# omroot/DeepLearningInAssetPricing_PaperReplication

Measured on AMD Instinct MI355X. Metric: epochs/sec (3-phase GAN), higher is better.
Workload: dtype bf16; 1 GPU; model=Chen-Pelger-Zhu GAN: LSTM[4] + SDF FFN[64,64] + 8 tanh moments, global_batch=1, seq_len=240, panel=T=240/60/300 N=3000 F=46 M=178, bench_config=real, wide_layer0=False, models_per_gpu=1, parallelism=ensemble-dp1, backend=none

## Files before the change

csrc/engine.cpp:

```cpp
#include <cstdint>
#include <cstdlib>
#include <hip/hip_runtime.h>
#include <pybind11/numpy.h>
#include <pybind11/pybind11.h>
#include <pybind11/stl.h>

#include <execinfo.h>
#include <signal.h>
#include <sys/syscall.h>
#include <unistd.h>

#include <atomic>
#include <cmath>
#include <cstring>
#include <map>
#include <memory>
#include <mutex>
#include <stdexcept>
#include <string>
#include <vector>

#include <chrono>

#include "engine_plan.h"
// ... 137 lines not shown
    {
      hipDeviceProp_t prop;
      int dev = 0;
      HIP_OK(hipGetDevice(&dev));
      HIP_OK(hipGetDeviceProperties(&prop, dev));
      std::vector<uint32_t> mask((prop.multiProcessorCount + 31) / 32, 0u);
      for (int cu = 0; cu < prop.multiProcessorCount; ++cu) mask[cu / 32] |= 1u << (cu % 32);
      HIP_OK(hipExtStreamCreateWithCUMask(&st2_, (uint32_t)mask.size(), mask.data()));
    }
    own_st_ = st_;
    for (hipEvent_t& e : ev_) HIP_OK(hipEventCreateWithFlags(&e, hipEventDisableTiming));
    build_desc(F, M, nrnn, H, raw_macro_sdf, hidden, mom_hidden, K, dropout, normalize_w, weighted,
               residual, fp32);
    prog_.alloc((size_t)G * 3 * 16);
    esync_.alloc(64);
    d_desc_.alloc(sizeof(ModelDesc));
    HIP_LEGACY(hipMemcpy(d_desc_.p, &md_, sizeof(ModelDesc), hipMemcpyHostToDevice));
    models_.resize(G);
    for (int g = 0; g < G; ++g) {
      ModelState& S = models_[g];
      S.dropout = dropout;
      S.params.alloc(md_.P); S.grads.alloc(md_.P); S.m.alloc(md_.P); S.v.alloc(md_.P);
      S.snap_loss.alloc(md_.P); S.snap_sharpe.alloc(md_.P);
      S.gnorm.alloc(1); S.best.alloc(3); S.aux.alloc((size_t)2 * md_.md.aux_floats);
      S.hist.alloc((size_t)max_epochs_ * HIST_W);
      S.adam_step.alloc(2); S.drop_step.alloc(1); S.snap_flags.alloc(2); S.ep.alloc(2); S.upd_ctr.alloc(1);
      S.tail_ctr.alloc(lstm_tail_words());
      S.blob.alloc((size_t)2 * md_.md.blob_frags * 512 * xw());
      S.blob0.alloc((size_t)std::max(1, md_.md.b0_frags) * 512 * xw());
      S.wproj.alloc((size_t)(md_.proj_mp + 2) * md_.proj_np);
// ... 846 lines not shown
  }
  EvalPass eval_pass(int phase) const {
    EvalPass ep;
    ep.gram = gram_eval() && plan_ev_[phase];
    return ep;
  }
  const LossJob* loss_tab(int phase, bool gram) const {
    return gram ? as<LossJob>(j_loss_gram_[phase]) : as<LossJob>(j_loss_train_[phase]);
  }
  double capture_s_ = 0.0;
  double host_launch_s_ = 0.0;
  long host_launch_n_ = 0;
  DevBuf<char> j_rnn_all_;
  DevBuf<int> prog_;
  DevBuf<int> esync_;
  int cap_train_ = 0, cap_eval_ = 0, cap_all_ = 0;
  int tail_cap_ = 0;
  PhasePlan plan_[4];
  static int fused_grid(int want, int njobs, int cap) {
    if (cap <= 0 || njobs <= 0) return 0;
    const int gx = std::min(want, cap / njobs - 1);
    return gx >= 16 ? gx : 0;
  }
  int eval_grid() const {
    int gx = std::max(gx_fwd_[1], gx_fwd_[2]);
    if (k_.eval_gx > 0) gx = std::min(gx, k_.eval_gx);
    return gx;
  }
  int train_fwd_grid(int phase) const { return phase == 2 ? gx_fwd_[0] : gx_fwd13_; }
  int ne_per_model() const { return G_ > 0 && n_eval_jobs_ % G_ == 0 ? n_eval_jobs_ / G_ : 0; }
// ... 12 lines not shown
      p.eval_gx_solo = eval_gx;
      p.eval_fusable = eval_fusable;
      const int gx = fused_grid(train_fwd_grid(phase), G_, cap_train_);
      p.fused_fwd = (phase != 2 || k_.fused_p2) && overlap && fits(splits_[0].T) && gx > 0;
      p.train_gx = p.fused_fwd ? gx : 0;
      p.selfproj = p.fused_fwd && k_.self_proj && !train_mom(phase);
      const int gxa = cap_all_ > 0 && ne > 0 ? std::min(train_fwd_grid(phase), cap_all_ / G_ - 1 - ne) : 0;
      p.eval_in_fwd = k_.eval_in_fwd && phase != 2 && ne > 0 && p.fused_fwd && fits(tmax_fwd_all()) && gxa >= 16;
      p.all_gx = p.eval_in_fwd ? gxa : 0;
      p.sep_eval = k_.eval_sep && phase != 2 && p.fused_fwd && eval_fusable;
      p.tail_fused = k_.fused_tail && !xs_on_ && phase != 2 && have0 && lstm_tail_supported(md_, splits_[0].T);
      const int nadam = (md_.P_sdf + ADAM_PB - 1) / ADAM_PB;
      p.adam_in_tail = k_.tail_adam != 0 && !safe_mode_ && p.tail_fused && packs && tail_cap_ > 0 &&
                       2 * G_ * nadam <= tail_cap_;
      p.split_graphs = k_.split_graphs && !safe_mode_ && p.adam_in_tail && (p.sep_eval || p.eval_in_fwd);
      p.mom_tail = phase == 2 && k_.mom_tail && !xs_on_ && packs && have0 && mom_tail_supported(md_, splits_[0].T);
      p.p2_lstm_cached = phase == 2 && k_.p2_lstm_cache && md_.nrnn > 0 && (md_.nrnn == 1 || md_.dropout == 0.f) &&
                         !xs_on_;
      plan_[phase] = p;
    }
  }
  RunMode run_mode(int phase) const {
    const PhasePlan& p = plan_[phase];
    RunMode m;
    m.pipe = phase != 2 && n_eval_jobs_ > 0 && pipeline_;
    m.split = m.pipe && p.split_graphs;
    m.sep = m.split && p.sep_eval;
    m.tail_adam = m.split || (m.pipe && p.eval_in_fwd && k_.tail_adam == 2 && p.adam_in_tail);
    return m;
  }
 public:
  double capture_seconds() const { return capture_s_; }
  bool fused_fwd(int phase) const { return phase >= 1 && phase <= 3 && plan_[phase].fused_fwd; }
  void reset_prog_errors() {
    sync();
    std::vector<int> h((size_t)G_ * 3 * 16);
    HIP_LEGACY(hipMemcpy(h.data(), prog_.p, h.size() * sizeof(int), hipMemcpyDeviceToHost));
    for (int k = 0; k < 3 * G_; ++k) h[16 * k + 1] = 0;
    HIP_LEGACY(hipMemcpy(prog_.p, h.data(), h.size() * sizeof(int), hipMemcpyHostToDevice));
    for (ModelState& S : models_) {
      HIP_LEGACY(hipMemset(S.tail_ctr.p, 0, S.tail_ctr.n * sizeof(int)));
      HIP_LEGACY(hipMemset(S.upd_ctr.p, 0, S.upd_ctr.n * sizeof(int)));
    }
    HIP_LEGACY(hipMemset(esync_.p, 0, esync_.n * sizeof(int)));
  }
  py::dict fused_info() const {
    py::dict d;
    const RunMode m = run_mode(1);
    d["cap_train"] = cap_train_; d["cap_eval"] = cap_eval_;
    for (int ph = 1; ph <= 3; ++ph) d[("train_gx_p" + std::to_string(ph)).c_str()] = plan_[ph].train_gx;
    d["eval_gx_solo"] = plan_[1].eval_gx_solo;
    d["cap_all"] = cap_all_;
    d["tail_cap"] = tail_cap_;
    for (int ph = 1; ph <= 3; ph += 2) {
      d[("eval_in_fwd_p" + std::to_string(ph)).c_str()] = plan_[ph].eval_in_fwd;
      d[("all_gx_p" + std::to_string(ph)).c_str()] = plan_[ph].all_gx;
    }
    d["eval_per_model"] = ne_per_model();
    d["fused_tail"] = plan_[1].tail_fused;
    d["mom_tail"] = plan_[2].mom_tail;
    d["p2_lstm_cached"] = plan_[2].p2_lstm_cached;
    d["adam_in_tail"] = m.tail_adam && plan_[1].eval_in_fwd;
    d["split_graphs"] = m.split;
    d["eval_sep"] = m.sep;
    d["host_launch_us_per_epoch"] = host_launch_n_ ? 1e6 * host_launch_s_ / host_launch_n_ : 0.0;
    d["bwd_nfine"] = nfine_; d["bwd_fpw"] = fpw_;
    d["fused_pack"] = inv_code_.p != nullptr;
    d["bwd_lds_fpw1"] = (long)mlp_bwd_lds_bytes(md_.md, slab_stride(), 1);
    d["bwd_lds_fpw4"] = (long)mlp_bwd_lds_bytes(md_.md, slab_stride(), 4);
    return d;
  }
  int prog_timeouts() {
    sync();
    std::vector<int> h((size_t)G_ * 3 * 16);
    HIP_LEGACY(hipMemcpy(h.data(), prog_.p, h.size() * sizeof(int), hipMemcpyDeviceToHost));
    int n = 0;
    for (int k = 0; k < 3 * G_; ++k) n += h[16 * k + 1];
    return n;
  }
// ... 450 lines not shown
  }
  void join_eval_gram() {
    if (!eval_gram_pending_) return;
    HIP_OK(hipStreamWaitEvent(st_, ev_[EV_GRAM], 0));
    eval_gram_pending_ = false;
  }

  void rebuild_jobs() {
    HTRACE("rebuild_jobs");
    sync();
    if (st2_) HIP_OK(hipStreamSynchronize(st2_));
    for (ModelState& S : models_) {
      HIP_LEGACY(hipMemset(S.tail_ctr.p, 0, S.tail_ctr.n * sizeof(int)));
      HIP_LEGACY(hipMemset(S.upd_ctr.p, 0, S.upd_ctr.n * sizeof(int)));
    }
    tail_cap_ = splits_[0].set && lstm_tail_supported(md_, splits_[0].T) ? lstm_tail_capacity(md_, splits_[0].T) : 0;
    for (auto& kv : graphs_) retire_graph_exec(kv.second, st_);
    graphs_.clear();
    fwd_tables_.clear();
    j_mlp_bwd_dh_.free();
    {
      const int want = k_.bwd_fpw;
      const int tps = std::max(md_.tps_s, md_.tps_m);
      fpw_ = (want == 4 && !md_.tbwd && mlp_bwd_fpw_fits(md_.md, md_.KS1, slab_stride(), tps, 4)) ? 4 : 1;
      gx_bwd_ = nfine_ / fpw_;
    }
    std::vector<RnnJob> rt, re;
    std::vector<LossJob> le, led;
    std::vector<MlpJob> me;
    std::vector<FinJob> fj;
// ... 298 lines not shown
      HTRACE("launch_mlp_fwd_zx");
      launch_mlp_fwd_zx(as<MlpJob>(j_mlp_eval_), n_eval_jobs_, std::max(1, k_.zx_gx / n_eval_jobs_), md_.md, md_.WMB, st);
    } else {
      if (md_.md.wide)
        launch_proj0(as<WideJob>(j_wide_eval_), n_eval_jobs_, std::max(gx_proj_[1], gx_proj_[2]), md_.md, md_.WMB, st);
      HTRACE("launch_mlp_fwd");
      if (fused_eval(ep))
        launch_mlp_fwd_rnn(as<MlpJob>(j_mlp_eval_), as<RnnJob>(j_rnn_eval_), dd(), n_eval_jobs_, plan_[1].eval_gx_solo,
                           md_.md, md_.KS1, md_.WMB, md_.H, md_.nrnn, tmax_eval_, st, k_.h_cache, 0, ep.selfproj);
      else
        launch_mlp_fwd(as<MlpJob>(j_mlp_eval_), n_eval_jobs_, eval_grid(), md_.md, md_.KS1, md_.WMB, st, k_.h_cache);
    }
    const LossJob* le = as<LossJob>(ep.gram ? j_loss_eval_ : j_loss_eval_dense_);
    HTRACE("launch_period_fwd");
    period_fwd(le, n_eval_jobs_, tmax_eval_, st, false, 6);
    if (ep.gram) {
      HTRACE("launch_period_bwd(eval)");
      launch_period_bwd(le, n_eval_jobs_, tmax_eval_, st);
    } else {
      HTRACE("launch_asset");
      launch_asset(le, n_eval_jobs_, nmax_eval_, md_.K, st);
      if (xs_on_) { launch_xs_loss_sums(le, n_eval_jobs_, st); xs_call("loss", 6, st); }
    }
    HTRACE("launch_job_metrics");
    launch_job_metrics(le, n_eval_jobs_, st);
  }
  void enqueue_eval_solo(int phase) {
    EvalPass ep = eval_pass(phase);
    ep.solo = true;
    enqueue_eval(st_, ep);
  }
  void enqueue_epoch_end(int phase, int ignore_epoch, float sel, hipStream_t st, int signal = 0) {
    HTRACE("launch_epoch_end");
    launch_epoch_end(as<EpochJob>(j_epoch_[phase]), G_, phase, ignore_epoch, sel, md_.residual_factor,
                     md_.P, st, signal);
  }
  void enqueue_epoch(int phase, float lr, int ignore_epoch, float sel, bool lstm_once) {
    TrainPass tp = epoch_pass(phase, lr);
    tp.mom_adam = plan_[phase].mom_tail;
    tp.lstm_once = lstm_once;
    enqueue_train_grads(tp);
    if (!tp.mom_adam) enqueue_update(phase, lr);
    if (phase != 2) enqueue_eval_solo(phase);
    enqueue_epoch_end(phase, ignore_epoch, sel, st_);
  }
  void enqueue_head(int phase, float lr, int part) {
    TrainPass tp = epoch_pass(phase, lr);
    tp.part = part;
    enqueue_train_grads(tp);
    enqueue_dropmask(phase, 1, st_);
// ... 10 lines not shown
    tp.esig = sep ? nullptr : esync_.p;
    enqueue_train_grads(tp);
  }
  void enqueue_eval_split(int phase, int ignore_epoch, float sel) {
    EvalPass ep = eval_pass(phase);
    if (plan_[phase].sep_eval) {
      HTRACE("launch_wait_gen");
      launch_wait_gen(as<UpdJob>(j_upd_), G_, k_.spin_limit, st2_);
      ep.sep = true;
      ep.selfproj = k_.self_proj && k_.h_cache;
      if (!ep.selfproj) launch_proj(as<RnnJob>(j_rnn_eval_), n_eval_jobs_, tmax_eval_, dd(), md_, st2_, !k_.h_cache);
    } else {
      HTRACE("launch_wait_count");
      launch_wait_count(esync_.p, ne_per_model() * G_, k_.spin_limit, prog_.p, G_, st2_);
    }
    enqueue_eval_towers(st2_, ep);
    enqueue_dropmask(phase, 1, st2_);
    enqueue_epoch_end(phase, ignore_epoch, sel, st2_, 1);
  }
  void enqueue_pipe(int phase, float lr, int ignore_epoch, float sel) {
    HIP_OK(hipEventRecord(ev_[EV_FORK], st_));
    HIP_OK(hipStreamWaitEvent(st2_, ev_[EV_FORK], 0));
    TrainPass tp = epoch_pass(phase, lr);
    tp.premasked = true;
    const EvalPass ep = eval_pass(phase);
    if (plan_[phase].eval_in_fwd) {
      const bool ta = run_mode(phase).tail_adam;
      tp.eval_rnn = tp.mark_fwd = tp.tail_metrics = true;
      tp.tail_adam = ta ? 2 : 0;
      enqueue_train_grads(tp);
      HIP_OK(hipStreamWaitEvent(st2_, ev_[EV_FWD], 0));
      enqueue_eval_towers(st2_, ep);
      if (ta) {
        enqueue_dropmask(phase, 1, st2_);
        enqueue_epoch_end(phase, ignore_epoch, sel, st2_, 1);
        HIP_OK(hipEventRecord(ev_[EV_JOIN], st2_));
        HIP_OK(hipStreamWaitEvent(st_, ev_[EV_JOIN], 0));
        return;
      }
      enqueue_epoch_end(phase, ignore_epoch, sel, st2_);
      enqueue_dropmask(phase, 1, st2_);
    } else {
      tp.eval_prologue = st2_;
      tp.defer_metrics = true;
      enqueue_train_grads(tp);
      enqueue_eval_towers(st2_, ep);
// ... 212 lines not shown
```

csrc/engine_plan.h:

```cpp
#pragma once
#include <hip/hip_runtime.h>

#include <algorithm>
#include <cstdlib>

inline int grid_per_model(int one, int lo, int G) { return std::max(lo, one / std::max(1, G)); }

inline int env_int(const char* name, int dflt) {
  const char* v = std::getenv(name);
  return v && *v ? std::atoi(v) : dflt;
}

struct Knobs {
  bool rnn_overlap;
  bool rnn_overlap_eval;
  bool fused_p2;
  bool eval_in_fwd;
  bool eval_sep;
  bool self_proj;
  bool fused_tail;
  bool mom_tail;
  int tail_adam;
  bool split_graphs;
  int unroll;
  bool p2_lstm_cache;
  bool train_gram_side;
  bool h_cache;
  bool gram;
  int gram_plan;
  bool fused_pack;
  int prog_mode;
  unsigned spin_limit;
  int fused_cap;
  bool wide;
  int tps;
  bool tbwd;
  int eval_gx;
  bool zx_eval, zx_train;
// ... 7 lines not shown
  bool pp_global;
};

inline Knobs read_knobs(int G, bool fp32) {
  Knobs k{};
  k.rnn_overlap = env_int("DLAP_RNN_OVERLAP", 1) != 0;
  k.rnn_overlap_eval = env_int("DLAP_RNN_OVERLAP_EVAL", 0) != 0;
  k.fused_p2 = env_int("DLAP_FUSED_PHASE2", 0) != 0;
  k.eval_in_fwd = env_int("DLAP_EVAL_IN_FWD", 1) != 0;
  k.eval_sep = env_int("DLAP_EVAL_SEP", 0) != 0;
  k.self_proj = env_int("DLAP_SELF_PROJ", 1) != 0;
  k.fused_tail = env_int("DLAP_FUSED_TAIL", 1) != 0;
  k.mom_tail = env_int("DLAP_MOM_TAIL", 1) != 0;
  k.tail_adam = env_int("DLAP_TAIL_ADAM", 1);
  k.split_graphs = env_int("DLAP_SPLIT_GRAPHS", 1) != 0;
  k.unroll = std::max(1, env_int("DLAP_UNROLL", 8));
  k.p2_lstm_cache = env_int("DLAP_P2_LSTM_CACHE", 1) != 0;
  k.train_gram_side = env_int("DLAP_TRAIN_GRAM_SIDE", 0) != 0;
  k.h_cache = env_int("DLAP_H_CACHE", 1) != 0;
  k.gram = env_int("DLAP_GRAM", 1) != 0;
  k.gram_plan = env_int("DLAP_GRAM_PLAN", 1);
  k.fused_pack = env_int("DLAP_FUSED_PACK", 1) != 0;
  k.prog_mode = env_int("DLAP_PROG_MODE", 1);
  k.spin_limit = (unsigned)env_int("DLAP_PROG_SPIN_LIMIT", 1 << 22);
  k.fused_cap = env_int("DLAP_FUSED_CAP", -1);
  k.wide = env_int("DLAP_WIDE", 0) != 0;
  k.tps = env_int("DLAP_TPS", 1);
  k.tbwd = env_int("DLAP_TBWD", 1) != 0;
  k.eval_gx = env_int("DLAP_EVAL_GX", grid_per_model(256, 64, G));
  k.zx_eval = !fp32 && env_int("DLAP_ZX_EVAL", 1) != 0;
// ... 7 lines not shown
  k.bwd_fpw = env_int("DLAP_BWD_FPW", 1);
  k.pp_global = env_int("DLAP_PP_GLOBAL", 0) != 0;
  return k;
}

struct PhasePlan {
  bool fused_fwd = false;
  int train_gx = 0;
  bool eval_in_fwd = false;
  int all_gx = 0;
  bool selfproj = false;
  bool sep_eval = false;
  bool tail_fused = false;
  bool adam_in_tail = false;
  bool split_graphs = false;
  bool mom_tail = false;
  bool p2_lstm_cached = false;
  bool eval_fusable = false;
  int eval_gx_solo = 0;
};

struct RunMode {
  bool pipe = false;
  bool split = false;
  bool sep = false;
  bool tail_adam = false;
};

struct TrainPass {
  explicit TrainPass(int phase_, float lr_ = 0.f) : phase(phase_), lr(lr_) {}
// ... 7 lines not shown
  int* esig = nullptr;
  hipStream_t eval_prologue = nullptr;
  bool lstm_once = false;
  bool mark_fwd = false;
  bool defer_metrics = false;
  bool tail_metrics = false;
  int tail_adam = 0;
  bool mom_adam = false;
};

struct EvalPass {
  bool gram = false;
  bool solo = false;
  bool sep = false;
  bool selfproj = false;
};
```

csrc/k_loss.hip:

```cpp
#include <cstdlib>

#include "common.h"
#include "loss.h"
#include "loss_dev.h"

__device__ long long g_loss_ts[4];

#define PER_NT 512
#define PER_RB 8
__global__ __launch_bounds__(PER_NT) void k_period_fwd(const LossJob* __restrict__ jobs, int store_wn, int stage) {
  const LossJob& J = jobs[blockIdx.y];
  const int t = blockIdx.x;
  if (stage <= 1 && J.prog_reset && t == 0 && threadIdx.x == 0) gp(J.prog_reset)[0] = 0;
  if (t >= J.T) return;
  __shared__ float red[PER_NT / 64];
  const int N = J.N;
  const float invN = gp(J.invNt)[t];
  auto finish = [&](float s_wr, float s_abs, float s_ww) {
    const float p = J.weighted ? s_wr * invN * J.Nbar : s_wr;
    gp(J.P)[t] = p;
    gp(J.sdfv)[t] = 1.f + p;
    if (gp(J.port)) gp(J.port)[t] = s_wr / fmaxf(s_abs, 1e-8f);
    if (gp(J.rstat)) {
      gp(J.rstat)[4 * t + 0] = s_ww;
// ... 295 lines not shown
        v *= invT;
        gp(J.Eu)[i] = v;
        if (gp(J.dEu)) gp(J.dEu)[i] = J.coef_u * v;
        lu = v * v;
      }
    }
  }
  lc = block_sum<256>(lc, lred);
  lu = block_sum<256>(lu, lred);
  if (threadIdx.x == 0) {
    gp(J.part)[2 * blockIdx.x + 0] = lc;
    gp(J.part)[2 * blockIdx.x + 1] = lu;
  }
}

DLAP_DEV float gram_period(const LossJob& J, int t, double* redd) {
  const int T = J.T;
  const size_t T2 = (size_t)T * T;
  const auto G = gp(J.G) + (size_t)t * T;
  const auto sv = gp(J.sdfv);
  const bool cond = J.h != nullptr;
  double vc = 0.0, vu = 0.0;
  for (int u = threadIdx.x; u < T; u += PER_NT) {
    const double s = (double)sv[u];
    if (cond) vc += G[u] * s;
    vu += G[T2 + u] * s;
  }
  if (cond) vc = block_sum_d<PER_NT>(vc, redd);
  vu = block_sum_d<PER_NT>(vu, redd);
  if (threadIdx.x == 0) {
    const double st = (double)sv[t];
    gp(J.gpart)[2 * t + 0] = cond ? st * vc : 0.0;
    gp(J.gpart)[2 * t + 1] = st * vu;
  }
  if (J.phase == 1) return (float)((double)J.coef_u * vu);
  if (J.phase == 2 || J.phase == 3) return (float)((double)J.coef_c * vc);
  return 0.f;
}

template <bool METRICS>
__global__ __launch_bounds__(PER_NT) void k_period_bwd(const LossJob* __restrict__ jobs) {
  const LossJob& J = jobs[blockIdx.y];
  const int t = blockIdx.x;
  __shared__ float red[PER_NT / 64];
  if constexpr (METRICS) {
    __shared__ float ret[DLAP_MAX_T];
    if (t == (int)gridDim.x - 1) { job_metrics_body<PER_NT>(J, red, ret, g_loss_ts); return; }
  }
  if (t >= J.T) return;
  const int N = J.N, K = J.K;
  const size_t base = (size_t)t * N;
  const int r0 = gp(J.row_ptr)[t], r1 = gp(J.row_ptr)[t + 1];
  DLAP_ASSERT(0 <= r0 && r0 <= r1 && r1 <= J.R);
  float sg = 0.f;
  if (J.gram) {
    __shared__ double redd[PER_NT / 64];
    sg = gram_period(J, t, redd);
    if (J.phase == 0) return;
  }
  if (r1 == r0) return;
  const auto rowti = gp(J.rowti);
  const auto Rc = gp(J.Rc);
  const auto invT = gp(J.invT);
  auto row_g = [&](int i) -> float {
    if (J.phase == 1) return gp(J.dEu)[i];
    const auto hp = gp(J.h) + (base + i) * K;
    const auto de = gp(J.dE) + (size_t)i * K;
    float g = 0.f;
    for (int k = 0; k < K; ++k) g += de[k] * hp[k];
    return g;
  };
  constexpr int RB = 4;
// ... 199 lines not shown
```

csrc/k_update.hip:

```cpp
#include "common.h"
#include "layout.h"
#include "update.h"
#include "loss.h"
#include "finalize.h"
#include "pack_dev.h"

__global__ __launch_bounds__(256) void k_finalize(const FinJob* __restrict__ jobs,
                                                  const ModelDesc* __restrict__ md, int phase,
                                                  int slab_stride, int b0) {
  finalize_block(jobs[blockIdx.y], md, phase, slab_stride, blockIdx.x + b0);
}

void launch_finalize(const FinJob* jobs, int njobs, const ModelDesc* md, const ModelDesc& mh,
                     int phase, int slab_stride, int tmax, hipStream_t st, int part) {
  const bool mom = phase == 2;
  const int ntile = mom ? mh.ntile_m : mh.ntile_s;
  const int D = mom ? 64 : (mh.nrnn > 0 ? mh.Dm : 0);
  const int nslab = ntile * 64 + (SLAB_EXTRA + 63) / 64, nper = D > 0 ? tmax : 0;
  const int b0 = part == 2 ? nslab : 0;
  const int nb = part == 1 ? nslab : part == 2 ? nper : nslab + nper;
  if (nb == 0) return;
  hipLaunchKernelGGL(k_finalize, dim3(nb, njobs), dim3(256), 0, st, jobs, md, phase, slab_stride, b0);
  HIP_OK(hipGetLastError());
}
// ... 121 lines not shown
                   float lr, hipStream_t st, bool fused) {
  const int n = phase == 2 ? mh.P - mh.P_sdf : mh.P_sdf;
  hipLaunchKernelGGL(k_adam, dim3((n + ADAM_PB - 1) / ADAM_PB, njobs), dim3(256), 0, st, jobs, md, phase,
                     lr);
  HIP_OK(hipGetLastError());
  if (fused) return;
  hipLaunchKernelGGL(k_pack, dim3(pack_blocks_of(mh), njobs), dim3(256), 0, st, jobs, md,
                     phase == 2 ? 2 : 1);
  HIP_OK(hipGetLastError());
}

#define EPOCH_END_THREADS 1024
__global__ __launch_bounds__(EPOCH_END_THREADS) void k_epoch_end(const EpochJob* __restrict__ jobs, int phase,
                                                   int ignore_epoch, float sel, float res_factor, int P,
                                                   int signal) {
  const EpochJob& J = jobs[blockIdx.x];
  __shared__ int dec[2];
  if (threadIdx.x == 0) {
    const bool hv = phase != 2 && J.sc_valid, ht = hv && J.sc_test;
    float tr[SC_NSCAL], va[SC_NSCAL], te[SC_NSCAL];
#pragma unroll
    for (int c = 0; c < SC_NSCAL; ++c) {
      tr[c] = gp(J.sc_train)[c];
      va[c] = hv ? gp(J.sc_valid)[c] : 0.f;
      te[c] = ht ? gp(J.sc_test)[c] : 0.f;
    }
    const int ep = gp(J.ep)[0], ep_ph = gp(J.ep)[1];
    const bool poisoned = prog_poisoned(J.prog);
    const float gn = gp(J.gnorm)[0];
    const float best0 = gp(J.best)[0], best1 = gp(J.best)[1], best2 = gp(J.best)[2];
    __shared__ float spill[HIST_W];
    float* row = ep < J.max_ep ? gp(J.hist) + (size_t)ep * HIST_W : spill;
    const float lres = tr[SC_LRES] * res_factor;
    float tloss;
    if (phase == 1) tloss = tr[SC_LUNC] + lres;
    else if (phase == 2) tloss = -tr[SC_LCOND] + lres;
    else tloss = tr[SC_LCOND] + lres;
    float r[HIST_W];
#pragma unroll
    for (int c = 0; c < HIST_W; ++c) r[c] = __builtin_nanf("");
    r[H_PHASE] = (float)phase;
    r[H_TRAIN_LOSS] = tloss;
    r[H_TRAIN_SHARPE] = tr[SC_TRAIN_SHARPE];
    r[H_TRAIN_LUNC] = phase == 2 ? 0.f : tr[SC_LUNC];
    r[H_TRAIN_LCOND] = phase == 1 ? 0.f : tr[SC_LCOND];
    r[H_TRAIN_LRES] = tr[SC_LRES];
    r[H_GNORM] = gn;
    int up_loss = 0, up_sr = 0;
    if (poisoned) {
#pragma unroll
      for (int c = 1; c < HIST_W; ++c) r[c] = __builtin_nanf("");
    } else if (hv) {
      const float vloss = phase == 1 ? va[SC_LUNC] : va[SC_LCOND];
      r[H_VALID_LOSS] = vloss;
      r[H_VALID_SHARPE] = va[SC_SHARPE];
      r[H_VALID_LUNC] = va[SC_LUNC];
      r[H_VALID_LCOND] = va[SC_LCOND];
      r[H_VALID_MDD] = va[SC_MDD];
      r[H_VALID_MEAN] = va[SC_MEAN];
      r[H_VALID_STD] = va[SC_STD];
      if (ht) {
        r[H_TEST_LOSS] = phase == 1 ? te[SC_LUNC] : te[SC_LCOND];
        r[H_TEST_SHARPE] = te[SC_SHARPE];
        r[H_TEST_LUNC] = te[SC_LUNC];
        r[H_TEST_LCOND] = te[SC_LCOND];
        r[H_TEST_MDD] = te[SC_MDD];
        r[H_TEST_MEAN] = te[SC_MEAN];
        r[H_TEST_STD] = te[SC_STD];
      }
      if (ep_ph > ignore_epoch) {
        if (vloss < best0) { gp(J.best)[0] = vloss; up_loss = 1; }
        const float s = sel * va[SC_SHARPE];
        if (s > best1) { gp(J.best)[1] = s; up_sr = 1; }
      }
    } else if (phase == 2) {
      const float lc = tr[SC_LCOND];
      if (lc > best2) { gp(J.best)[2] = lc; up_loss = 1; }
    }
    r[H_BEST_LOSS] = (float)up_loss;
    r[H_BEST_SR] = (float)up_sr;
#pragma unroll
    for (int c = 0; c < HIST_W; ++c) row[c] = r[c];
    if (up_loss) gp(J.snap_flags)[0] = 1;
    if (up_sr) gp(J.snap_flags)[1] = 1;
    gp(J.ep)[0] = ep + 1;
    gp(J.ep)[1] = ep_ph + 1;
    dec[0] = up_loss;
    dec[1] = up_sr;
  }
  __syncthreads();
  auto copy = [&](float* dst) {
    const auto src = gp(J.params);
    const auto d = gp(dst);
    const int P4 = ((reinterpret_cast<uintptr_t>(J.params) | reinterpret_cast<uintptr_t>(dst)) & 15) ? 0 : P >> 2;
    constexpr int U = 8;
    for (int i0 = threadIdx.x; i0 < P4; i0 += U * EPOCH_END_THREADS) {
      f32x4 v[U];
#pragma unroll
      for (int u = 0; u < U; ++u) {
        const int i = i0 + u * EPOCH_END_THREADS;
        v[u] = i < P4 ? ld4(src + 4 * i) : zero4();
      }
#pragma unroll
      for (int u = 0; u < U; ++u) {
        const int i = i0 + u * EPOCH_END_THREADS;
        if (i < P4) *(DLAP_GLOBAL f32x4*)(d + 4 * i) = v[u];
      }
    }
    for (int i = 4 * P4 + threadIdx.x; i < P; i += EPOCH_END_THREADS) d[i] = src[i];
  };
  if (dec[0]) copy(J.snap_loss);
  if (dec[1]) copy(J.snap_sharpe);
  if (signal) {
    __syncthreads();
    if (threadIdx.x == 0) {
      __builtin_amdgcn_fence(__ATOMIC_RELEASE, "agent");
      __hip_atomic_fetch_add(J.eval_gen, 1, __ATOMIC_RELAXED, __HIP_MEMORY_SCOPE_AGENT);
    }
  }
}

__global__ __launch_bounds__(64) void k_begin_phase(const EpochJob* __restrict__ jobs, int njobs) {
  const int g = blockIdx.x * 64 + threadIdx.x;
  if (g >= njobs) return;
  const EpochJob& J = jobs[g];
  gp(J.best)[0] = INFINITY;
  gp(J.best)[1] = -INFINITY;
  gp(J.best)[2] = -INFINITY;
  gp(J.snap_flags)[0] = 0;
  gp(J.snap_flags)[1] = 0;
  gp(J.ep)[1] = 0;
}

void launch_begin_phase(const EpochJob* jobs, int njobs, hipStream_t st) {
// ... 11 lines not shown
```

csrc/loss_dev.h:

```cpp
#pragma once
#include "common.h"
#include "loss.h"

DLAP_DEV void residual_stats(const LossJob& J, float& lres, float& inv_b, float& n1) {
  float a = 0.f, b = 0.f, c1 = 0.f, c2 = 0.f;
  for (int t = 0; t < J.T; ++t) {
    const float n = gp(J.Nt)[t];
    if (n < 2.f) continue;
    const float ww = gp(J.rstat)[4 * t + 0], rw = gp(J.rstat)[4 * t + 1], rr = gp(J.RR)[t];
    b += rr / n; c2 += 1.f;
    if (ww > 1e-8f) { a += (rr - rw * rw / ww) / n; c1 += 1.f; }
  }
  if (c1 == 0.f) { lres = 0.f; inv_b = 0.f; n1 = 0.f; return; }
  const float B = fmaxf(b / c2, 1e-8f);
  lres = (a / c1) / B;
  inv_b = 1.f / B;
  n1 = c1;
}

#define AF_S 16
DLAP_DEV int asset_red_blocks(const LossJob& J) {
  return J.asset_full ? (J.N + AF_S - 1) / AF_S : (J.N * (J.h ? J.K + 1 : 1) + 255) >> 8;
}

template <int NT>
DLAP_DEV double block_sum_d(double v, double* red) {
#pragma unroll
  for (int o = 32; o > 0; o >>= 1) v += __shfl_xor(v, o, 64);
  __syncthreads();
  if ((threadIdx.x & 63) == 0) red[threadIdx.x >> 6] = v;
  __syncthreads();
  double s = 0.0;
#pragma unroll
  for (int i = 0; i < NT / 64; ++i) s += red[i];
  return s;
}

template <int NT>
DLAP_DEV double block_sum_d(double v, double* red);

template <int NT>
DLAP_DEV void local_loss_sums(const LossJob& J, float& a, float& b, float* red) {
  const int nblk = asset_red_blocks(J);
  a = 0.f; b = 0.f;
  for (int k = threadIdx.x; k < nblk; k += NT) { a += gp(J.part)[2 * k]; b += gp(J.part)[2 * k + 1]; }
  a = block_sum<NT>(a, red);
  b = block_sum<NT>(b, red);
}

template <int NT>
// ... 100 lines not shown
```

csrc/update.h:

```cpp
#pragma once
#include "common.h"

struct ModelDesc;

#define PACK_FAN 4
#define ADAM_PB 1024
#define TAIL_CNT 0
#define TAIL_FLAG 32
#define TAIL_DONE 64
#define TAIL_ARRIVE 96
#define TAIL_EVGEN 128
#define TAIL_ARRIVE2 160
#define TAIL_ADONE 192
#define TAIL_UPDGEN 224
#define TAIL_UPDSEEN 256
#define TAIL_WORDS 288

struct FinJob {
  const float* slab;
  float* grads;
  const int* row_ptr;
  const float* u;
  float* dpp;
  const float* v;
// ... 79 lines not shown
void launch_lstm_tail(const UpdJob* ujobs, const FinJob* fjobs, int njobs, const ModelDesc* md, const ModelDesc& mh,
                      int T, int slab_stride, hipStream_t st, const LossJob* ljobs = nullptr, int adam = 0,
                      float lr = 0.f, int phase = 1);
bool mom_tail_supported(const ModelDesc& mh, int T);
void launch_pack(float* const* params_unused, const UpdJob* jobs, int njobs, const ModelDesc* md,
                 const ModelDesc& mh, hipStream_t st);
int pack_total(const ModelDesc& mh);
void pack_index_host(const ModelDesc& mh, int* src);
void launch_set_int(int* p, int v, hipStream_t st);
void launch_begin_phase(const EpochJob* jobs, int njobs, hipStream_t st);
void launch_wait_count(int* cnt, int per, unsigned limit, int* prog, int nmodels, hipStream_t st);
void launch_wait_gen(const UpdJob* jobs, int njobs, unsigned limit, hipStream_t st);
void launch_gen_sync(const UpdJob* jobs, int njobs, hipStream_t st);
void launch_epoch_end(const EpochJob* jobs, int njobs, int phase, int ignore_epoch, float sel,
                      float res_factor, int P, hipStream_t st, int signal = 0);
```

Baseline: 7154 model-epochs/s.

## Fuse eval gram backward, metrics, dropout mask and epoch-end into one tail kernel

Adds a k_eval_tail kernel that runs the eval-side gram period pass, then uses last-block-arrives atomic counters to compute per-job metrics, generate the next dropout masks, and run the epoch-end bookkeeping in a single launch. It is on by default when G==1 and replaces several separate eval-stream launches (period bwd, metrics, dropmask, epoch_end). The goal is to cut launch and dependency overhead on the serial tail of each epoch. In exchange it adds device-side counters that must be reset, atomic-store ordering requirements, and more complex control flow. The epoch-end body is factored into a shared device function.

Result: no change. 7210 model-epochs/s (median of 6 runs) (+0.8%).

```diff
diff --git a/csrc/engine.cpp b/csrc/engine.cpp
--- a/csrc/engine.cpp
+++ b/csrc/engine.cpp
@@ -175,6 +175,7 @@
                residual, fp32);
     prog_.alloc((size_t)G * 3 * 16);
     esync_.alloc(64);
+    evt_ctr_.alloc((size_t)eval_tail_ctr_words(2 * G, G));
     d_desc_.alloc(sizeof(ModelDesc));
     HIP_LEGACY(hipMemcpy(d_desc_.p, &md_, sizeof(ModelDesc), hipMemcpyHostToDevice));
     models_.resize(G);
@@ -1051,6 +1052,7 @@
   DevBuf<char> j_rnn_all_;
   DevBuf<int> prog_;
   DevBuf<int> esync_;
+  DevBuf<int> evt_ctr_;
   int cap_train_ = 0, cap_eval_ = 0, cap_all_ = 0;
   int tail_cap_ = 0;
   PhasePlan plan_[4];
@@ -1093,6 +1095,7 @@
       p.adam_in_tail = k_.tail_adam != 0 && !safe_mode_ && p.tail_fused && packs && tail_cap_ > 0 &&
                        2 * G_ * nadam <= tail_cap_;
       p.split_graphs = k_.split_graphs && !safe_mode_ && p.adam_in_tail && (p.sep_eval || p.eval_in_fwd);
+      p.eval_tail = k_.eval_tail && phase != 2 && gram_eval() && !xs_on_ && ne > 0;
       p.mom_tail = phase == 2 && k_.mom_tail && !xs_on_ && packs && have0 && mom_tail_supported(md_, splits_[0].T);
       p.p2_lstm_cached = phase == 2 && k_.p2_lstm_cache && md_.nrnn > 0 && (md_.nrnn == 1 || md_.dropout == 0.f) &&
                          !xs_on_;
@@ -1122,6 +1125,7 @@
       HIP_LEGACY(hipMemset(S.upd_ctr.p, 0, S.upd_ctr.n * sizeof(int)));
     }
     HIP_LEGACY(hipMemset(esync_.p, 0, esync_.n * sizeof(int)));
+    HIP_LEGACY(hipMemset(evt_ctr_.p, 0, evt_ctr_.n * sizeof(int)));
   }
   py::dict fused_info() const {
     py::dict d;
@@ -1142,6 +1146,7 @@
     d["adam_in_tail"] = m.tail_adam && plan_[1].eval_in_fwd;
     d["split_graphs"] = m.split;
     d["eval_sep"] = m.sep;
+    d["eval_tail"] = plan_[1].eval_tail;
     d["host_launch_us_per_epoch"] = host_launch_n_ ? 1e6 * host_launch_s_ / host_launch_n_ : 0.0;
     d["bwd_nfine"] = nfine_; d["bwd_fpw"] = fpw_;
     d["fused_pack"] = inv_code_.p != nullptr;
@@ -1622,6 +1627,7 @@
       HIP_LEGACY(hipMemset(S.tail_ctr.p, 0, S.tail_ctr.n * sizeof(int)));
       HIP_LEGACY(hipMemset(S.upd_ctr.p, 0, S.upd_ctr.n * sizeof(int)));
     }
+    HIP_LEGACY(hipMemset(evt_ctr_.p, 0, evt_ctr_.n * sizeof(int)));
     tail_cap_ = splits_[0].set && lstm_tail_supported(md_, splits_[0].T) ? lstm_tail_capacity(md_, splits_[0].T) : 0;
     for (auto& kv : graphs_) retire_graph_exec(kv.second, st_);
     graphs_.clear();
@@ -1950,6 +1956,7 @@
     const LossJob* le = as<LossJob>(ep.gram ? j_loss_eval_ : j_loss_eval_dense_);
     HTRACE("launch_period_fwd");
     period_fwd(le, n_eval_jobs_, tmax_eval_, st, false, 6);
+    if (ep.losses_open) return;
     if (ep.gram) {
       HTRACE("launch_period_bwd(eval)");
       launch_period_bwd(le, n_eval_jobs_, tmax_eval_, st);
@@ -1970,6 +1977,16 @@
     HTRACE("launch_epoch_end");
     launch_epoch_end(as<EpochJob>(j_epoch_[phase]), G_, phase, ignore_epoch, sel, md_.residual_factor,
                      md_.P, st, signal);
+  }
+  bool eval_tail_on(int phase, const EvalPass& ep) const { return plan_[phase].eval_tail && ep.gram && n_eval_jobs_ > 0; }
+  void enqueue_eval_tail(int phase, int ignore_epoch, float sel, hipStream_t st) {
+    HTRACE("launch_eval_tail");
+    const bool masks = dropmask_on(phase);
+    const int ntiles = (splits_[0].R + 31) / 32;
+    launch_eval_tail(as<LossJob>(j_loss_eval_), n_eval_jobs_, tmax_eval_, ne_per_model(), as<EpochJob>(j_epoch_[phase]),
+                     masks ? as<MlpJob>(j_mlp_train_[phase]) : nullptr, md_.md.nl_sdf,
+                     masks ? eval_tail_mask_blocks(ntiles, G_) : 0, evt_ctr_.p, phase, ignore_epoch, sel,
+                     md_.residual_factor, md_.P, 1, st);
   }
   void enqueue_epoch(int phase, float lr, int ignore_epoch, float sel, bool lstm_once) {
     TrainPass tp = epoch_pass(phase, lr);
@@ -2010,6 +2027,12 @@
       HTRACE("launch_wait_count");
       launch_wait_count(esync_.p, ne_per_model() * G_, k_.spin_limit, prog_.p, G_, st2_);
     }
+    if (eval_tail_on(phase, ep)) {
+      ep.losses_open = true;
+      enqueue_eval_towers(st2_, ep);
+      enqueue_eval_tail(phase, ignore_epoch, sel, st2_);
+      return;
+    }
     enqueue_eval_towers(st2_, ep);
     enqueue_dropmask(phase, 1, st2_);
     enqueue_epoch_end(phase, ignore_epoch, sel, st2_, 1);
@@ -2019,13 +2042,21 @@
     HIP_OK(hipStreamWaitEvent(st2_, ev_[EV_FORK], 0));
     TrainPass tp = epoch_pass(phase, lr);
     tp.premasked = true;
-    const EvalPass ep = eval_pass(phase);
+    EvalPass ep = eval_pass(phase);
     if (plan_[phase].eval_in_fwd) {
       const bool ta = run_mode(phase).tail_adam;
       tp.eval_rnn = tp.mark_fwd = tp.tail_metrics = true;
       tp.tail_adam = ta ? 2 : 0;
       enqueue_train_grads(tp);
       HIP_OK(hipStreamWaitEvent(st2_, ev_[EV_FWD], 0));
+      if (ta && eval_tail_on(phase, ep)) {
+        ep.losses_open = true;
+        enqueue_eval_towers(st2_, ep);
+        enqueue_eval_tail(phase, ignore_epoch, sel, st2_);
+        HIP_OK(hipEventRecord(ev_[EV_JOIN], st2_));
+        HIP_OK(hipStreamWaitEvent(st_, ev_[EV_JOIN], 0));
+        return;
+      }
       enqueue_eval_towers(st2_, ep);
       if (ta) {
         enqueue_dropmask(phase, 1, st2_);
diff --git a/csrc/engine_plan.h b/csrc/engine_plan.h
--- a/csrc/engine_plan.h
+++ b/csrc/engine_plan.h
@@ -22,6 +22,7 @@
   bool mom_tail;
   int tail_adam;
   bool split_graphs;
+  bool eval_tail;
   int unroll;
   bool p2_lstm_cache;
   bool train_gram_side;
@@ -59,6 +60,7 @@
   k.mom_tail = env_int("DLAP_MOM_TAIL", 1) != 0;
   k.tail_adam = env_int("DLAP_TAIL_ADAM", 1);
   k.split_graphs = env_int("DLAP_SPLIT_GRAPHS", 1) != 0;
+  k.eval_tail = env_int("DLAP_EVAL_TAIL", G == 1 ? 1 : 0) != 0;
   k.unroll = std::max(1, env_int("DLAP_UNROLL", 8));
   k.p2_lstm_cache = env_int("DLAP_P2_LSTM_CACHE", 1) != 0;
   k.train_gram_side = env_int("DLAP_TRAIN_GRAM_SIDE", 0) != 0;
@@ -96,6 +98,7 @@
   bool tail_fused = false;
   bool adam_in_tail = false;
   bool split_graphs = false;
+  bool eval_tail = false;
   bool mom_tail = false;
   bool p2_lstm_cached = false;
   bool eval_fusable = false;
@@ -133,4 +136,5 @@
   bool solo = false;
   bool sep = false;
   bool selfproj = false;
+  bool losses_open = false;
 };
diff --git a/csrc/epoch_dev.h b/csrc/epoch_dev.h
--- /dev/null
+++ b/csrc/epoch_dev.h
@@ -0,0 +1,110 @@
+#pragma once
+#include "common.h"
+#include "update.h"
+#include "loss.h"
+#include "pack_dev.h"
+
+DLAP_DEV void epoch_end_body(const EpochJob& J, int phase, int ignore_epoch, float sel, float res_factor, int P,
+                             int signal, int nt, int* dec, float* spill) {
+  if (threadIdx.x == 0) {
+    const bool hv = phase != 2 && J.sc_valid, ht = hv && J.sc_test;
+    float tr[SC_NSCAL], va[SC_NSCAL], te[SC_NSCAL];
+#pragma unroll
+    for (int c = 0; c < SC_NSCAL; ++c) {
+      tr[c] = gp(J.sc_train)[c];
+      va[c] = hv ? gp(J.sc_valid)[c] : 0.f;
+      te[c] = ht ? gp(J.sc_test)[c] : 0.f;
+    }
+    const int ep = gp(J.ep)[0], ep_ph = gp(J.ep)[1];
+    const bool poisoned = prog_poisoned(J.prog);
+    const float gn = gp(J.gnorm)[0];
+    const float best0 = gp(J.best)[0], best1 = gp(J.best)[1], best2 = gp(J.best)[2];
+    float* row = ep < J.max_ep ? gp(J.hist) + (size_t)ep * HIST_W : spill;
+    const float lres = tr[SC_LRES] * res_factor;
+    float tloss;
+    if (phase == 1) tloss = tr[SC_LUNC] + lres;
+    else if (phase == 2) tloss = -tr[SC_LCOND] + lres;
+    else tloss = tr[SC_LCOND] + lres;
+    float r[HIST_W];
+#pragma unroll
+    for (int c = 0; c < HIST_W; ++c) r[c] = __builtin_nanf("");
+    r[H_PHASE] = (float)phase;
+    r[H_TRAIN_LOSS] = tloss;
+    r[H_TRAIN_SHARPE] = tr[SC_TRAIN_SHARPE];
+    r[H_TRAIN_LUNC] = phase == 2 ? 0.f : tr[SC_LUNC];
+    r[H_TRAIN_LCOND] = phase == 1 ? 0.f : tr[SC_LCOND];
+    r[H_TRAIN_LRES] = tr[SC_LRES];
+    r[H_GNORM] = gn;
+    int up_loss = 0, up_sr = 0;
+    if (poisoned) {
+#pragma unroll
+      for (int c = 1; c < HIST_W; ++c) r[c] = __builtin_nanf("");
+    } else if (hv) {
+      const float vloss = phase == 1 ? va[SC_LUNC] : va[SC_LCOND];
+      r[H_VALID_LOSS] = vloss;
+      r[H_VALID_SHARPE] = va[SC_SHARPE];
+      r[H_VALID_LUNC] = va[SC_LUNC];
+      r[H_VALID_LCOND] = va[SC_LCOND];
+      r[H_VALID_MDD] = va[SC_MDD];
+      r[H_VALID_MEAN] = va[SC_MEAN];
+      r[H_VALID_STD] = va[SC_STD];
+      if (ht) {
+        r[H_TEST_LOSS] = phase == 1 ? te[SC_LUNC] : te[SC_LCOND];
+        r[H_TEST_SHARPE] = te[SC_SHARPE];
+        r[H_TEST_LUNC] = te[SC_LUNC];
+        r[H_TEST_LCOND] = te[SC_LCOND];
+        r[H_TEST_MDD] = te[SC_MDD];
+        r[H_TEST_MEAN] = te[SC_MEAN];
+        r[H_TEST_STD] = te[SC_STD];
+      }
+      if (ep_ph > ignore_epoch) {
+        if (vloss < best0) { gp(J.best)[0] = vloss; up_loss = 1; }
+        const float s = sel * va[SC_SHARPE];
+        if (s > best1) { gp(J.best)[1] = s; up_sr = 1; }
+      }
+    } else if (phase == 2) {
+      const float lc = tr[SC_LCOND];
+      if (lc > best2) { gp(J.best)[2] = lc; up_loss = 1; }
+    }
+    r[H_BEST_LOSS] = (float)up_loss;
+    r[H_BEST_SR] = (float)up_sr;
+#pragma unroll
+    for (int c = 0; c < HIST_W; ++c) row[c] = r[c];
+    if (up_loss) gp(J.snap_flags)[0] = 1;
+    if (up_sr) gp(J.snap_flags)[1] = 1;
+    gp(J.ep)[0] = ep + 1;
+    gp(J.ep)[1] = ep_ph + 1;
+    dec[0] = up_loss;
+    dec[1] = up_sr;
+  }
+  __syncthreads();
+  auto copy = [&](float* dst) {
+    const auto src = gp(J.params);
+    const auto d = gp(dst);
+    const int P4 = ((reinterpret_cast<uintptr_t>(J.params) | reinterpret_cast<uintptr_t>(dst)) & 15) ? 0 : P >> 2;
+    constexpr int U = 8;
+    for (int i0 = threadIdx.x; i0 < P4; i0 += U * nt) {
+      f32x4 v[U];
+#pragma unroll
+      for (int u = 0; u < U; ++u) {
+        const int i = i0 + u * nt;
+        v[u] = i < P4 ? ld4(src + 4 * i) : zero4();
+      }
+#pragma unroll
+      for (int u = 0; u < U; ++u) {
+        const int i = i0 + u * nt;
+        if (i < P4) *(DLAP_GLOBAL f32x4*)(d + 4 * i) = v[u];
+      }
+    }
+    for (int i = 4 * P4 + threadIdx.x; i < P; i += nt) d[i] = src[i];
+  };
+  if (dec[0]) copy(J.snap_loss);
+  if (dec[1]) copy(J.snap_sharpe);
+  if (signal) {
+    __syncthreads();
+    if (threadIdx.x == 0) {
+      __builtin_amdgcn_fence(__ATOMIC_RELEASE, "agent");
+      __hip_atomic_fetch_add(J.eval_gen, 1, __ATOMIC_RELAXED, __HIP_MEMORY_SCOPE_AGENT);
+    }
+  }
+}
diff --git a/csrc/k_eval_tail.hip b/csrc/k_eval_tail.hip
--- /dev/null
+++ b/csrc/k_eval_tail.hip
@@ -0,0 +1,97 @@
+#include <algorithm>
+
+#include "common.h"
+#include "loss.h"
+#include "loss_dev.h"
+#include "mlp.h"
+#include "update.h"
+#include "epoch_dev.h"
+
+#define EVT_STRIDE 32
+
+int eval_tail_ctr_words(int njobs, int nmodels) { return (njobs + nmodels) * EVT_STRIDE; }
+
+int eval_tail_mask_blocks(int ntiles, int nmodels) {
+  const int cap = std::max(16, 512 / std::max(1, nmodels));
+  return std::max(1, std::min((ntiles + PER_NT / 64 - 1) / (PER_NT / 64), cap));
+}
+
+DLAP_DEV bool arrive_last(int* ctr, int target, unsigned* s_ord) {
+  asm volatile("s_waitcnt vmcnt(0)" ::: "memory");
+  __syncthreads();
+  if (threadIdx.x == 0)
+    *s_ord = __hip_atomic_fetch_add(reinterpret_cast<unsigned*>(ctr), 1u, __ATOMIC_RELAXED, __HIP_MEMORY_SCOPE_AGENT);
+  __syncthreads();
+  if ((*s_ord + 1u) % (unsigned)target != 0u) return false;
+  if (threadIdx.x < 64) {
+    asm volatile("" ::: "memory");
+    __builtin_amdgcn_fence(__ATOMIC_ACQUIRE, "agent");
+    asm volatile("s_waitcnt vmcnt(0)" ::: "memory");
+  }
+  __syncthreads();
+  return true;
+}
+
+__global__ __launch_bounds__(PER_NT) void k_eval_tail(const LossJob* __restrict__ jobs, int njobs, int tmax, int ne,
+                                                      const EpochJob* __restrict__ ejobs,
+                                                      const MlpJob* __restrict__ mjobs, int nl_sdf, int nmb, int* ctr,
+                                                      int phase, int ignore_epoch, float sel, float res_factor, int P,
+                                                      int signal) {
+  __shared__ double redd[PER_NT / 64];
+  __shared__ float red[4];
+  __shared__ float ret[DLAP_MAX_T];
+  __shared__ float spill[HIST_W];
+  __shared__ unsigned s_ord;
+  __shared__ int dec[2];
+  const int nper = njobs * tmax;
+  int g, nt;
+  if ((int)blockIdx.x < nper) {
+    const int j = blockIdx.x / tmax, t = blockIdx.x - j * tmax;
+    const LossJob& J = jobs[j];
+    if (t >= J.T) return;
+    gram_period<true>(J, t, redd);
+    if (!arrive_last(ctr + EVT_STRIDE * j, J.T, &s_ord)) return;
+    if (threadIdx.x >= 256) return;
+    job_metrics_body<256>(J, red, ret, nullptr);
+    g = j / ne;
+    nt = 256;
+  } else {
+    const int mb = (int)blockIdx.x - nper;
+    g = mb / nmb;
+    const int b = mb - g * nmb;
+    nt = PER_NT;
+    const MlpJob& M = mjobs[g];
+    if (M.dropout > 0.f) {
+      const int ntiles = (M.R + 31) >> 5;
+      const uint32_t step = (M.step ? (uint32_t)*gp(M.step) : 0u) + 1u;
+      const uint32_t thr16 = (uint32_t)(M.dropout * 65536.f + 0.5f);
+      const int lane = threadIdx.x & 63, q = lane >> 4, wave = threadIdx.x >> 6;
+      const auto base = gp(const_cast<uint32_t*>(M.gbits)) + (size_t)(step & 1u) * M.gb_half + lane;
+      for (int tile = b * (PER_NT / 64) + wave; tile < ntiles; tile += nmb * (PER_NT / 64)) {
+        uint32_t rowmix[2];
+#pragma unroll
+        for (int h = 0; h < 2; ++h) {
+          const int r = tile * 32 + 16 * h + (lane & 15);
+          const int2 ti = gp(M.rowti)[min(r, M.R - 1)];
+          rowmix[h] = row_mix(r < M.R ? (uint32_t)(ti.x * M.N + ti.y) : 0xFFFFFFFFu);
+        }
+        const auto dst = base + (size_t)tile * nl_sdf * 64;
+        for (int l = 0; l < nl_sdf; ++l)
+          __hip_atomic_store(dst + 64 * l, keep_word<4>(dropout_key(M.seed, step, l), rowmix, thr16, q),
+                             __ATOMIC_RELAXED, __HIP_MEMORY_SCOPE_AGENT);
+      }
+    }
+  }
+  if (!arrive_last(ctr + EVT_STRIDE * (njobs + g), ne + nmb, &s_ord)) return;
+  epoch_end_body(ejobs[g], phase, ignore_epoch, sel, res_factor, P, signal, nt, dec, spill);
+}
+
+void launch_eval_tail(const LossJob* jobs, int njobs, int tmax, int ne, const EpochJob* ejobs, const MlpJob* mjobs,
+                      int nl_sdf, int nmb, int* ctr, int phase, int ignore_epoch, float sel, float res_factor,
+                      int P, int signal, hipStream_t st) {
+  if (!mjobs) nmb = 0;
+  const int nmodels = njobs / ne;
+  hipLaunchKernelGGL(k_eval_tail, dim3(njobs * tmax + nmodels * nmb), dim3(PER_NT), 0, st, jobs, njobs, tmax, ne,
+                     ejobs, mjobs, nl_sdf, nmb, ctr, phase, ignore_epoch, sel, res_factor, P, signal);
+  HIP_OK(hipGetLastError());
+}
diff --git a/csrc/k_loss.hip b/csrc/k_loss.hip
--- a/csrc/k_loss.hip
+++ b/csrc/k_loss.hip
@@ -6,7 +6,6 @@
 
 __device__ long long g_loss_ts[4];
 
-#define PER_NT 512
 #define PER_RB 8
 __global__ __launch_bounds__(PER_NT) void k_period_fwd(const LossJob* __restrict__ jobs, int store_wn, int stage) {
   const LossJob& J = jobs[blockIdx.y];
@@ -333,30 +332,6 @@
   }
 }
 
-DLAP_DEV float gram_period(const LossJob& J, int t, double* redd) {
-  const int T = J.T;
-  const size_t T2 = (size_t)T * T;
-  const auto G = gp(J.G) + (size_t)t * T;
-  const auto sv = gp(J.sdfv);
-  const bool cond = J.h != nullptr;
-  double vc = 0.0, vu = 0.0;
-  for (int u = threadIdx.x; u < T; u += PER_NT) {
-    const double s = (double)sv[u];
-    if (cond) vc += G[u] * s;
-    vu += G[T2 + u] * s;
-  }
-  if (cond) vc = block_sum_d<PER_NT>(vc, redd);
-  vu = block_sum_d<PER_NT>(vu, redd);
-  if (threadIdx.x == 0) {
-    const double st = (double)sv[t];
-    gp(J.gpart)[2 * t + 0] = cond ? st * vc : 0.0;
-    gp(J.gpart)[2 * t + 1] = st * vu;
-  }
-  if (J.phase == 1) return (float)((double)J.coef_u * vu);
-  if (J.phase == 2 || J.phase == 3) return (float)((double)J.coef_c * vc);
-  return 0.f;
-}
-
 template <bool METRICS>
 __global__ __launch_bounds__(PER_NT) void k_period_bwd(const LossJob* __restrict__ jobs) {
   const LossJob& J = jobs[blockIdx.y];
@@ -374,7 +349,7 @@
   float sg = 0.f;
   if (J.gram) {
     __shared__ double redd[PER_NT / 64];
-    sg = gram_period(J, t, redd);
+    sg = gram_period<false>(J, t, redd);
     if (J.phase == 0) return;
   }
   if (r1 == r0) return;
diff --git a/csrc/k_update.hip b/csrc/k_update.hip
--- a/csrc/k_update.hip
+++ b/csrc/k_update.hip
@@ -4,6 +4,7 @@
 #include "loss.h"
 #include "finalize.h"
 #include "pack_dev.h"
+#include "epoch_dev.h"
 
 __global__ __launch_bounds__(256) void k_finalize(const FinJob* __restrict__ jobs,
                                                   const ModelDesc* __restrict__ md, int phase,
@@ -159,110 +160,9 @@
 __global__ __launch_bounds__(EPOCH_END_THREADS) void k_epoch_end(const EpochJob* __restrict__ jobs, int phase,
                                                    int ignore_epoch, float sel, float res_factor, int P,
                                                    int signal) {
-  const EpochJob& J = jobs[blockIdx.x];
   __shared__ int dec[2];
-  if (threadIdx.x == 0) {
-    const bool hv = phase != 2 && J.sc_valid, ht = hv && J.sc_test;
-    float tr[SC_NSCAL], va[SC_NSCAL], te[SC_NSCAL];
-#pragma unroll
-    for (int c = 0; c < SC_NSCAL; ++c) {
-      tr[c] = gp(J.sc_train)[c];
-      va[c] = hv ? gp(J.sc_valid)[c] : 0.f;
-      te[c] = ht ? gp(J.sc_test)[c] : 0.f;
-    }
-    const int ep = gp(J.ep)[0], ep_ph = gp(J.ep)[1];
-    const bool poisoned = prog_poisoned(J.prog);
-    const float gn = gp(J.gnorm)[0];
-    const float best0 = gp(J.best)[0], best1 = gp(J.best)[1], best2 = gp(J.best)[2];
-    __shared__ float spill[HIST_W];
-    float* row = ep < J.max_ep ? gp(J.hist) + (size_t)ep * HIST_W : spill;
-    const float lres = tr[SC_LRES] * res_factor;
-    float tloss;
-    if (phase == 1) tloss = tr[SC_LUNC] + lres;
-    else if (phase == 2) tloss = -tr[SC_LCOND] + lres;
-    else tloss = tr[SC_LCOND] + lres;
-    float r[HIST_W];
-#pragma unroll
-    for (int c = 0; c < HIST_W; ++c) r[c] = __builtin_nanf("");
-    r[H_PHASE] = (float)phase;
-    r[H_TRAIN_LOSS] = tloss;
-    r[H_TRAIN_SHARPE] = tr[SC_TRAIN_SHARPE];
-    r[H_TRAIN_LUNC] = phase == 2 ? 0.f : tr[SC_LUNC];
-    r[H_TRAIN_LCOND] = phase == 1 ? 0.f : tr[SC_LCOND];
-    r[H_TRAIN_LRES] = tr[SC_LRES];
-    r[H_GNORM] = gn;
-    int up_loss = 0, up_sr = 0;
-    if (poisoned) {
-#pragma unroll
-      for (int c = 1; c < HIST_W; ++c) r[c] = __builtin_nanf("");
-    } else if (hv) {
-      const float vloss = phase == 1 ? va[SC_LUNC] : va[SC_LCOND];
-      r[H_VALID_LOSS] = vloss;
-      r[H_VALID_SHARPE] = va[SC_SHARPE];
-      r[H_VALID_LUNC] = va[SC_LUNC];
-      r[H_VALID_LCOND] = va[SC_LCOND];
-      r[H_VALID_MDD] = va[SC_MDD];
-      r[H_VALID_MEAN] = va[SC_MEAN];
-      r[H_VALID_STD] = va[SC_STD];
-      if (ht) {
-        r[H_TEST_LOSS] = phase == 1 ? te[SC_LUNC] : te[SC_LCOND];
-        r[H_TEST_SHARPE] = te[SC_SHARPE];
-        r[H_TEST_LUNC] = te[SC_LUNC];
-        r[H_TEST_LCOND] = te[SC_LCOND];
-        r[H_TEST_MDD] = te[SC_MDD];
-        r[H_TEST_MEAN] = te[SC_MEAN];
-        r[H_TEST_STD] = te[SC_STD];
-      }
-      if (ep_ph > ignore_epoch) {
-        if (vloss < best0) { gp(J.best)[0] = vloss; up_loss = 1; }
-        const float s = sel * va[SC_SHARPE];
-        if (s > best1) { gp(J.best)[1] = s; up_sr = 1; }
-      }
-    } else if (phase == 2) {
-      const float lc = tr[SC_LCOND];
-      if (lc > best2) { gp(J.best)[2] = lc; up_loss = 1; }
-    }
-    r[H_BEST_LOSS] = (float)up_loss;
-    r[H_BEST_SR] = (float)up_sr;
-#pragma unroll
-    for (int c = 0; c < HIST_W; ++c) row[c] = r[c];
-    if (up_loss) gp(J.snap_flags)[0] = 1;
-    if (up_sr) gp(J.snap_flags)[1] = 1;
-    gp(J.ep)[0] = ep + 1;
-    gp(J.ep)[1] = ep_ph + 1;
-    dec[0] = up_loss;
-    dec[1] = up_sr;
-  }
-  __syncthreads();
-  auto copy = [&](float* dst) {
-    const auto src = gp(J.params);
-    const auto d = gp(dst);
-    const int P4 = ((reinterpret_cast<uintptr_t>(J.params) | reinterpret_cast<uintptr_t>(dst)) & 15) ? 0 : P >> 2;
-    constexpr int U = 8;
-    for (int i0 = threadIdx.x; i0 < P4; i0 += U * EPOCH_END_THREADS) {
-      f32x4 v[U];
-#pragma unroll
-      for (int u = 0; u < U; ++u) {
-        const int i = i0 + u * EPOCH_END_THREADS;
-        v[u] = i < P4 ? ld4(src + 4 * i) : zero4();
-      }
-#pragma unroll
-      for (int u = 0; u < U; ++u) {
-        const int i = i0 + u * EPOCH_END_THREADS;
-        if (i < P4) *(DLAP_GLOBAL f32x4*)(d + 4 * i) = v[u];
-      }
-    }
-    for (int i = 4 * P4 + threadIdx.x; i < P; i += EPOCH_END_THREADS) d[i] = src[i];
-  };
-  if (dec[0]) copy(J.snap_loss);
-  if (dec[1]) copy(J.snap_sharpe);
-  if (signal) {
-    __syncthreads();
-    if (threadIdx.x == 0) {
-      __builtin_amdgcn_fence(__ATOMIC_RELEASE, "agent");
-      __hip_atomic_fetch_add(J.eval_gen, 1, __ATOMIC_RELAXED, __HIP_MEMORY_SCOPE_AGENT);
-    }
-  }
+  __shared__ float spill[HIST_W];
+  epoch_end_body(jobs[blockIdx.x], phase, ignore_epoch, sel, res_factor, P, signal, EPOCH_END_THREADS, dec, spill);
 }
 
 __global__ __launch_bounds__(64) void k_begin_phase(const EpochJob* __restrict__ jobs, int njobs) {
diff --git a/csrc/loss_dev.h b/csrc/loss_dev.h
--- a/csrc/loss_dev.h
+++ b/csrc/loss_dev.h
@@ -34,6 +34,38 @@
 #pragma unroll
   for (int i = 0; i < NT / 64; ++i) s += red[i];
   return s;
+}
+
+#define PER_NT 512
+template <bool WT>
+DLAP_DEV float gram_period(const LossJob& J, int t, double* redd) {
+  const int T = J.T;
+  const size_t T2 = (size_t)T * T;
+  const auto G = gp(J.G) + (size_t)t * T;
+  const auto sv = gp(J.sdfv);
+  const bool cond = J.h != nullptr;
+  double vc = 0.0, vu = 0.0;
+  for (int u = threadIdx.x; u < T; u += PER_NT) {
+    const double s = (double)sv[u];
+    if (cond) vc += G[u] * s;
+    vu += G[T2 + u] * s;
+  }
+  if (cond) vc = block_sum_d<PER_NT>(vc, redd);
+  vu = block_sum_d<PER_NT>(vu, redd);
+  if (threadIdx.x == 0) {
+    const double st = (double)sv[t];
+    const double a = cond ? st * vc : 0.0, b = st * vu;
+    if constexpr (WT) {
+      __hip_atomic_store(gp(J.gpart) + 2 * t + 0, a, __ATOMIC_RELAXED, __HIP_MEMORY_SCOPE_AGENT);
+      __hip_atomic_store(gp(J.gpart) + 2 * t + 1, b, __ATOMIC_RELAXED, __HIP_MEMORY_SCOPE_AGENT);
+    } else {
+      gp(J.gpart)[2 * t + 0] = a;
+      gp(J.gpart)[2 * t + 1] = b;
+    }
+  }
+  if (J.phase == 1) return (float)((double)J.coef_u * vu);
+  if (J.phase == 2 || J.phase == 3) return (float)((double)J.coef_c * vc);
+  return 0.f;
 }
 
 template <int NT>
diff --git a/csrc/update.h b/csrc/update.h
--- a/csrc/update.h
+++ b/csrc/update.h
@@ -117,3 +117,9 @@
 void launch_gen_sync(const UpdJob* jobs, int njobs, hipStream_t st);
 void launch_epoch_end(const EpochJob* jobs, int njobs, int phase, int ignore_epoch, float sel,
                       float res_factor, int P, hipStream_t st, int signal = 0);
+struct MlpJob;
+int eval_tail_ctr_words(int njobs, int nmodels);
+int eval_tail_mask_blocks(int ntiles, int nmodels);
+void launch_eval_tail(const LossJob* jobs, int njobs, int tmax, int ne, const EpochJob* ejobs, const MlpJob* mjobs,
+                      int nl_sdf, int nmb, int* ctr, int phase, int ignore_epoch, float sel, float res_factor,
+                      int P, int signal, hipStream_t st);
```
